# shincling/DL4SS

Measured on AMD Instinct MI355X. Metric: mixtures/sec (8 kHz, 4 s, 2-spk WSJ0-shape) at 1/2/4/8 MI355X, higher is better.
Workload: dtype bf16; 1 GPU; C2: 2-spk pit BiLSTM-4L magnitude mask (EvalVer model), B=32/GPU, N=32000 (T=251,F=129); global_batch=32, seq_len=251, parallelism=dp1, precision=bf16, loss=pit, launch=hip-graph, step=mix+STFT+fwd+loss+bwd+allreduce+Adam

## Files before the change

dl4ss_amd/_lib.py:

```python
import ctypes
import os

import torch

_HERE = os.path.dirname(os.path.abspath(__file__))
LIB_PATH = os.environ.get("DL4SS_LIB", os.path.join(_HERE, "libdl4ss_hip.so"))

P = ctypes.c_void_p
I = ctypes.c_int
LL = ctypes.c_longlong
F = ctypes.c_float
U = ctypes.c_uint

SIGNATURES = {
    "dl4ss_stft_fwd": [P, LL, I, I, I, I, P, P, P],
    "dl4ss_stft_fwd_ex": [P, LL, I, I, I, I, P, P, P, LL, LL, P],
    "dl4ss_istft": [P, LL, I, I, I, I, P, P],
    "dl4ss_mix_sources": [P, P, I, I, I, P, P, P, P],
    "dl4ss_gemm": [I, I, I, I, I, P, LL, P, LL, P, LL, P, I, F, I, I, P],
    "dl4ss_f32_to_bf16": [P, P, LL, P],
    "dl4ss_f32_to_bf16_2d": [P, LL, I, I, P, LL, P],
    "dl4ss_f32_to_bf16_hilo": [P, LL, I, I, P, LL, I, I, U, P],
    "dl4ss_birnn_bias_reduce": [I, I, I, I, P, P, P, P],
    "dl4ss_birnn_bias_reduce_ex": [I, I, I, I, P, P, P, F, P],
# ... 31 lines not shown
    "dl4ss_attn_dot_nblk": [I],
    "dl4ss_attn_dot_fwd": [P, P, I, I, I, I, I, P, P],
    "dl4ss_attn_dot_bwd": [P, P, I, P, P, I, I, I, I, P, P, P, P],
    "dl4ss_top_k_mask": [P, I, I, F, I, P, P, P, P],
    "dl4ss_attn_dot_fwd_ex": [P, P, I, I, I, I, I, P, LL, P],
    "dl4ss_classifier_select": [P, I, I, F, I, P, I, P, P, P, P],
    "dl4ss_mask_split": [P, P, LL, P, P, P],
    "dl4ss_time_mean": [P, I, I, I, P, P],
    "dl4ss_bss_corr": [P, I, I, I, I, P, P],
    "dl4ss_mix_sources_ex": [P, P, P, I, I, I, P, P, P, P],
    "dl4ss_mix_sources_rot": [P, P, P, P, I, I, I, P, P, P, P],
    "dl4ss_f32_to_bf16_2d_multi": [I, P, P, P, P, P, P, P],
    "dl4ss_mask_attn_loss_bf16v": [I, I, I, I, I, I, I, P, P, P, LL, P, LL, LL, P, F, F, P, P, LL, P, P, P, P, P],
    "dl4ss_bss_gram": [P, I, I, I, I, P, P, P, P],
    "dl4ss_adam_guarded": [P, P, P, P, LL, F, F, F, F, I, P, P, P],
    "dl4ss_adam_guarded_dp": [P, P, P, P, LL, F, F, F, F, I, P, P, P, P],
    "dl4ss_adam_guarded_dp_scaled": [P, P, P, P, LL, F, F, F, F, I, P, P, F, P, P],
    "dl4ss_adam_guarded_dp_scaled_bf16": [P, P, P, P, LL, F, F, F, F, I, P, P, F, P, I, P, P, P, P, P, P],
    "dl4ss_status_flag": [P, P, P],
    "dl4ss_birnn_plan_info": [I, I, I, I, I, P],
    "dl4ss_debug_set_spin_limit": [ctypes.c_uint],
    "dl4ss_debug_set_place_force": [ctypes.c_int],
    "dl4ss_debug_set_rnn_max_wg": [ctypes.c_int],
    "dl4ss_attn_align_nblk": [I],
    "dl4ss_attn_align_part_floats": [I, I, I],
    "dl4ss_attn_align_fwd": [P, P, I, P, P, P, I, I, I, P, LL, P],
    "dl4ss_attn_align_bwd": [P, P, I, P, P, P, P, I, I, I, P, P, LL, P, P, P, P, P],
    "dl4ss_mask_attn_align_loss": [I, I, I, I, I, I, P, P, P, P, P, P, LL, P, LL, LL, P, F, F, P, P, P, LL, P, P, P],
    "dl4ss_attn_align_finalize": [P, LL, I, I, I, I, P, P, P, P, P, P, P],
    "dl4ss_cls_head_fwd": [P, P, P, I, I, I, P, P, P],
    "dl4ss_cls_head_loss_bwd": [P, P, P, P, I, I, I, I, P, P, P, P, P, P],
    "dl4ss_disc_dims": [I, I, P],
    "dl4ss_disc_ws_bytes": [I, I, I],
    "dl4ss_disc_conv1_fwd": [I, P, P, P, I, I, I, P, P],
    "dl4ss_disc_conv64_fwd": [I, P, P, P, I, I, I, P, P],
    "dl4ss_disc_head_fwd": [I, P, P, P, I, I, I, P, P, P],
    "dl4ss_disc_head_bwd": [I, P, P, P, P, F, I, I, I, P, P, P, P, P, P],
    "dl4ss_disc_conv64_bwd": [I, P, P, P, P, I, I, I, P, P, P, P, LL, P],
    "dl4ss_disc_conv1_bwd": [I, P, P, P, P, I, I, I, P, P, P, P, LL, P],
}
RESTYPES = {"dl4ss_birnn_workspace_bytes": ctypes.c_longlong, "dl4ss_colsum_bf16_part_bytes": ctypes.c_longlong,
            "dl4ss_gemm_bf16_gl_ws_bytes": ctypes.c_longlong,
            "dl4ss_gemm_bf16_gl_grouped_ws_bytes": ctypes.c_longlong, "dl4ss_attn_nblk": ctypes.c_int,
            "dl4ss_attn_dot_nblk": ctypes.c_int, "dl4ss_attn_align_nblk": ctypes.c_int,
            "dl4ss_attn_align_part_floats": ctypes.c_longlong, "dl4ss_disc_ws_bytes": ctypes.c_longlong,
            "dl4ss_debug_set_spin_limit": None,
            "dl4ss_debug_set_place_force": None, "dl4ss_debug_set_rnn_max_wg": None}

_lib = None


def _load():
    global _lib
    if _lib is not None:
        return _lib
    if not os.path.exists(LIB_PATH):
        raise RuntimeError(
            f"dl4ss HIP library not found at {LIB_PATH}; run `python -m dl4ss_amd.build` "
            "(there is no CPU fallback)")
    lib = ctypes.CDLL(LIB_PATH)
    for name, argtypes in SIGNATURES.items():
        fn = getattr(lib, name)
        fn.argtypes = argtypes
        fn.restype = RESTYPES.get(name, ctypes.c_int)
    hip = ctypes.CDLL("libamdhip64.so")
    hip.hipGetErrorString.restype = ctypes.c_char_p
    hip.hipGetErrorString.argtypes = [ctypes.c_int]
    lib._hip = hip
    _lib = lib
    return lib
# ... 37 lines not shown
```

dl4ss_amd/csrc/birnn.hip:

```cpp
#include <cstdlib>
#include "birnn_common.h"

using namespace dl4ss_rnn;

namespace {

constexpr int DL4SS_RNN_WS_ZEROED = 0x100;
constexpr int DL4SS_RNN_DEFER_BIAS = 0x400;
constexpr int DL4SS_RNN_DGH_PAD8 = 0x200;
constexpr int DL4SS_RNN_DOUT_SLABS_MASK = 0x3000;
constexpr unsigned SPIN_LIMIT = 1u << 20;

struct Plan {
  int cell, H;
  int BC, NG, J, nchunk;
  int KP, KPL, HP, RP, RPL, KG, KGL;
  bool fwd_pk;
  bool bwd_pk;
  bool big;
  int R() const { return (cell == CELL_LSTM ? 4 : 3) * J; }
  int hm() const { return big ? HMAX_L : HMAX; }
  long long groups() const { return 2LL * nchunk; }
  size_t smem_fwd(bool mf) const { return fwd_lds_bytes(mf, hm(), BC, J, R(), HP, KP); }
  size_t smem_bwd(bool mf) const {
    int rpln, kgln;
    bwd_dims(RPL, KGL, rpln, kgln, big);
    return bwd_lds_bytes(mf, hm(), BC, J, NG, RP, RP * rpln, KG * kgln);
  }
  size_t smem_fwd_pk(bool xw) const { return fwd_pk_lds_bytes(BC, R(), xw); }
  size_t smem_bwd_pk() const { return bwd_pk_lds_bytes(BC, J); }
  long long zero_fwd(bool pk) const {
    return pk ? granule_bytes(groups(), PK_NCOPY, fwd_pk_copy_g(BC, NG)) : granule_bytes(groups(), GEN_NCOPY, fwd_copies_g(1, BC, H));
  }
  long long zero_bwd(bool pk) const {
    return pk ? granule_bytes(groups(), PK_NCOPY, bwd_pk_copy_g(BC, NG, H)) : granule_bytes(groups(), GEN_NCOPY, bwd_copies_g(1, BC, NG, H));
  }
};

int g_max_wg = 0;
int wg_limit() {
  if (g_max_wg > 0) return g_max_wg;
  static const int env = std::getenv("DL4SS_RNN_MAX_WG") ? std::atoi(std::getenv("DL4SS_RNN_MAX_WG")) : 0;
  if (env > 0) return env;
  const int cu = device_cu_count();
  return cu > 0 ? cu - cu / 16 : 240;
}

bool make_plan(int cell, int B, int H, Plan& p, bool mf = true, int max_wg = 0) {
  if (H > HMAX_L) return false;
  if (max_wg <= 0) max_wg = wg_limit();
  p.cell = cell;
  p.H = H;
  p.big = H > HMAX;
// ... 36 lines not shown
  return false;
}

bool act_cell_major(const Plan& p) { return p.fwd_pk && p.bwd_pk && p.BC >= 4; }

#if defined(RNN_STAMPS) || defined(RNN_TRACE)
u64* g_stamps = nullptr;
#endif

unsigned g_spin_limit = SPIN_LIMIT;
int g_place_force = 0;

void fill_args(RnnArgs& a, const Plan& p, int B, int T, int H) {
  a.spin_limit = g_spin_limit;
  a.place_force = g_place_force;
#if defined(RNN_STAMPS) || defined(RNN_TRACE)
  a.stamps = g_stamps;
#endif
  a.B = B; a.T = T; a.H = H; a.J = p.J; a.NG = p.NG; a.nchunk = p.nchunk;
  a.KP = p.KP; a.KPL = p.KPL; a.HP = p.HP;
  a.RP = p.RP; a.RPL = p.RPL; a.KG = p.KG; a.KGL = p.KGL;
}

int launch(bool fwd, bool mf, bool pk, const Plan& p, const RnnArgs& a, size_t smem, hipStream_t st) {
  const int grid = (int)(p.groups() * p.NG);
  const int e = fwd ? (pk ? launch_fwd_pk(a, p.cell, p.BC, grid, smem, st) : launch_fwd(a, p.cell, p.BC, mf, grid, smem, st))
                    : (pk ? launch_bwd_pk(a, p.cell, p.BC, grid, smem, st) : launch_bwd(a, p.cell, p.BC, mf, grid, smem, st));
  if (e) return e;
  DL4SS_CHECK_LAUNCH();
  return 0;
}

}

#if defined(RNN_STAMPS) || defined(RNN_TRACE)
DL4SS_API void dl4ss_debug_set_stamps(void* p) { g_stamps = reinterpret_cast<unsigned long long*>(p); }
#endif

constexpr int BIAS_JOBS_MAX = 8;
struct BiasJobs {
  int n, B, GH;
  float beta;
  const float* part[BIAS_JOBS_MAX];
  float* dbi[BIAS_JOBS_MAX];
  float* dbh[BIAS_JOBS_MAX];
};
__global__ __launch_bounds__(256) void bias_reduce_kernel(BiasJobs j) {
  const int i = blockIdx.x * 256 + threadIdx.x;
  const int B = j.B, GH = j.GH;
  if (i >= 2 * GH) return;
// ... 22 lines not shown
  }
  if (dbi) dbi[i] = j.beta != 0.f ? si + j.beta * dbi[i] : si;
  if (dbh) dbh[i] = j.beta != 0.f ? sh + j.beta * dbh[i] : sh;
}

static long long handoff_bytes(const Plan& p, int H);

static long long bias_part_bytes(const Plan& p, int H) {
  return p.big ? 0 : (long long)p.nchunk * p.BC * 2 * 2 * 4 * H * 4;
}

static long long workspace_bytes(const Plan& p, int H) { return handoff_bytes(p, H) + bias_part_bytes(p, H); }

static long long handoff_bytes(const Plan& p, int H) { return handoff_area_bytes(p.groups(), p.BC, p.NG, H, p.big); }

static long long ctl_offset(const Plan& p, int H) { return ctl_offset_bytes(p.groups(), p.BC, p.NG, H); }

DL4SS_API void dl4ss_debug_set_spin_limit(unsigned limit) { g_spin_limit = limit ? limit : SPIN_LIMIT; }

DL4SS_API void dl4ss_debug_set_place_force(int force) { g_place_force = force == 1 ? 1 : 0; }

DL4SS_API void dl4ss_debug_set_rnn_max_wg(int max_wg) { g_max_wg = max_wg > 0 ? max_wg : 0; }

DL4SS_API int dl4ss_birnn_plan_info(int cell, int B, int H, int precision, int max_wg, int* info) {
  DL4SS_REQUIRE(info && (cell == CELL_LSTM || cell == CELL_GRU) && B > 0 && H > 0);
  Plan p;
  if (!make_plan(cell, B, H, p, precision == 1, max_wg)) return (int)hipErrorInvalidValue;
  info[0] = p.BC; info[1] = p.NG; info[2] = p.J; info[3] = p.nchunk; info[4] = 2 * p.nchunk * p.NG;
  return 0;
}

static int split_batch(int cell, int B, int H, bool mf, Plan& ps) {
  int fit = 0;
  for (int b = B - 1; b >= 1 && !fit; --b)
    if (make_plan(cell, b, H, ps, mf)) fit = b;
  if (!fit) return 0;
  const int n = (B + fit - 1) / fit;
  const int bs = (B + n - 1) / n;
  return make_plan(cell, bs, H, ps, mf) ? bs : 0;
}

DL4SS_API long long dl4ss_birnn_workspace_bytes(int cell, int B, int H) {
  long long best = -1;
  for (bool mf : {false, true}) {
    Plan p;
    if (!make_plan(cell, B, H, p, mf) && (mf || split_batch(cell, B, H, mf, p) == 0)) continue;
// ... 198 lines not shown
  DL4SS_REQUIRE(dOut || !pk);
  DL4SS_REQUIRE(pk || (!dG_bf16 && !dGh_bf16 && !db_ih && !db_hh && dG && (cell == CELL_LSTM || dGh)));
  DL4SS_REQUIRE(dout_ns == 1 || (pk && p.BC == 4));
  if (!prezeroed) {
    hipError_t e = hipMemsetAsync(workspace, 0, p.zero_bwd(pk), st);
    if (e == hipSuccess && pk) e = hipMemsetAsync(static_cast<char*>(workspace) + ctl_offset(p, H), 0, CTL_BYTES, st);
    if (e != hipSuccess) return (int)e;
  }
  RnnArgs a{};
  fill_args(a, p, B, T, H);
  a.Whh = W_hh; a.act = const_cast<float*>(act); a.cs = const_cast<float*>(cs);
  a.hprev = const_cast<float*>(hprev); a.dOut = dOut; a.dOutB = dOut_bcast; a.dG = dG; a.dGh = dGh;
  a.dout_ns = dout_ns;
  a.dout_zs = (long long)B * T * 2 * H;
  a.dGb = reinterpret_cast<unsigned short*>(dG_bf16); a.dGhb = reinterpret_cast<unsigned short*>(dGh_bf16);
  const int GHc = (cell == CELL_LSTM ? 4 : 3) * H;
  a.ghb = dgh_pad8 ? (GHc + 7) / 8 * 8 : GHc;
  a.dbi = db_ih; a.dbh = db_hh;
  a.xbuf = reinterpret_cast<unsigned long long*>(workspace);
  a.gctl = pk ? reinterpret_cast<unsigned*>(static_cast<char*>(workspace) + ctl_offset(p, H)) : nullptr;
  const bool bias = pk && (db_ih || db_hh);
  a.dbpart = bias ? reinterpret_cast<float*>(static_cast<char*>(workspace) + handoff_bytes(p, H)) : nullptr;
  a.status = status;
  const int e = launch(false, mf, pk, p, a, pk ? p.smem_bwd_pk() : p.smem_bwd(mf), st);
  if (e || !bias || defer_bias) return e;
  const int GH = (cell == CELL_LSTM ? 4 : 3) * H;
  BiasJobs j{};
  j.n = 1; j.B = B; j.GH = GH; j.beta = 1.f; j.part[0] = a.dbpart; j.dbi[0] = db_ih; j.dbh[0] = db_hh;
  hipLaunchKernelGGL(bias_reduce_kernel, dim3((2 * GH + 255) / 256, 1), dim3(256), 0, st, j);
  return (int)hipGetLastError();
}

DL4SS_API int dl4ss_birnn_bias_reduce_ex(int cell, int B, int H, int n, void* const* workspaces,
                                         float* const* db_ih, float* const* db_hh, float beta, void* stream) {
  DL4SS_REQUIRE((cell == CELL_LSTM || cell == CELL_GRU) && B > 0 && H > 0 && n >= 1 && n <= BIAS_JOBS_MAX);
  DL4SS_REQUIRE(workspaces && db_ih && db_hh);
  Plan p;
  if (!make_plan(cell, B, H, p, true)) return (int)hipErrorInvalidValue;
  const int GH = (cell == CELL_LSTM ? 4 : 3) * H;
  BiasJobs j{};
  j.n = n; j.B = B; j.GH = GH; j.beta = beta;
  for (int i = 0; i < n; ++i) {
    DL4SS_REQUIRE(workspaces[i] && db_ih[i] && db_hh[i]);
    j.part[i] = reinterpret_cast<const float*>(static_cast<const char*>(workspaces[i]) + handoff_bytes(p, H));
    j.dbi[i] = db_ih[i];
    j.dbh[i] = db_hh[i];
  }
// ... 11 lines not shown
```

dl4ss_amd/csrc/birnn_bwd_pk.hip:

```cpp
#include "birnn_common.h"

namespace dl4ss_rnn {

__device__ __forceinline__ unsigned pack24(float v) {
  const unsigned u = __float_as_uint(v);
  return (u + 0x80u) >> 8;
}
__device__ __forceinline__ float unpack24(unsigned r) { return __uint_as_float(r << 8); }

template <int CELL, int BC, int NZ = 1>
__global__ __launch_bounds__(NT, 1) void rnn_bwd_pk_kernel(RnnArgs a) {
  constexpr int NGATE = CELL == CELL_LSTM ? 4 : 3;
  constexpr int BSL_Q = BC * 5;
  constexpr int BSL_G = 64 / BSL_Q > 0 ? 64 / BSL_Q : 1;
  constexpr int BSL_N = BWD_NPW * BSL_G < 16 ? BWD_NPW * BSL_G : 16;
  constexpr int GLK = (16 + BSL_N - 1) / BSL_N;
  static_assert(BSL_Q <= 64, "one (b, quad) item per lane");
  constexpr int WSPAN = bwd_wspan(HMAX);
  constexpr int MTWMAX = WSPAN / 16;
  constexpr int KSRMAX = (4 * JMAX + 31) / 32;
  constexpr int WSP = BWD_PK_WSP;
  const int H = a.H, T = a.T, J = a.J, NG = a.NG;
  const int R = NGATE * J;
  const int ngroups = 2 * a.nchunk;
  extern __shared__ __attribute__((aligned(16))) float smem[];
  int group, w;
  group_pk(a.gctl, NG, ngroups, a.spin_limit, a.status, smem, group, w);
  const int d = group / a.nchunk, chunk = group % a.nchunk;
  const int b0 = chunk * BC;
  const int j0 = w * J;
  const int tid = threadIdx.x;
  const int lane = tid & 63, wv = tid >> 6;
  const int GH = NGATE * H;
  const int AH = 4 * H;
  const int HG = ((H + 1) / 2 + 1) & ~1;

  unsigned short* sdgb = reinterpret_cast<unsigned short*>(smem);
  float* sdh = smem + 8 * SDG;
  float* wsc = sdh + ((16 * BC * J + 3) & ~3);
  constexpr int SOPP = bwd_pk_sopp(BC);
  constexpr int WSCN = bwd_pk_wsc_n(BC), SOPN = bwd_pk_sop_n(BC);
  float* sop = wsc + WSCN;
  for (int i = tid; i < 8 * SDG + 16 * BC * J; i += NT) smem[i] = 0.0f;

  const bool mv = wv < 4;
  bf16x8 afr[MTWMAX][KSRMAX];
#pragma unroll
  for (int t = 0; t < MTWMAX; ++t) {
    const int k = (wv * MTWMAX + t) * 16 + (lane & 15);
#pragma unroll
    for (int ks = 0; ks < KSRMAX; ++ks)
#pragma unroll
      for (int j = 0; j < 8; ++j) {
        const int rr = ks * 32 + 8 * (lane >> 4) + j;
        const int q = rr / J, u = rr % J;
        const bool ok = mv && k < H && rr < R && j0 + u < H;
        afr[t][ks][j] = (short)bf16_rne(ok ? a.Whh[((long long)d * GH + q * H + j0 + u) * H + k] : 0.0f);
      }
  }

  const int cb = tid >> 5, cu = tid & 31;
  const bool ct = tid < BC * 32 && cu < J;
  const int cj = j0 + cu;
  const int bg = b0 + cb;
  const bool cval = ct && cj < H && bg < a.B;
  float dc_next = 0.0f, dh_dir = 0.0f;
  const float doutb = (cval && a.dOutB) ? a.dOutB[(long long)bg * 2 * H + d * H + cj] : 0.0f;

  const int copy_g = NG * BC * HG;
  u64* xg = a.xbuf + (long long)group * PK_NCOPY * copy_g;
  const __amdgpu_buffer_rsrc_t xr = granule_rsrc(xg, (unsigned)(PK_NCOPY * copy_g * 8));
  __shared__ int s_wt;
  if (tid == 0) __hip_atomic_store(xg + PK_PLACE_COPY * copy_g + w, (1ull << 32) | xcc_id(), __ATOMIC_RELAXED, __HIP_MEMORY_SCOPE_AGENT);
  if (wv == WPOLL) {
    const bool wt = group_needs_write_through(xg + PK_PLACE_COPY * copy_g, NG, lane, a.spin_limit, a.status, a.place_force);
    if (lane == 0) s_wt = wt;
  }

  constexpr int WPF = WPOLL + BWD_NPW;
  constexpr int NPF = NT - WPF * 64;
  constexpr int NSL = CELL == CELL_LSTM ? 7 : 6;
// ... 115 lines not shown
      const int p = sl + BSL_N * g;
      on[g] = lane_on && p < NG;
      loff[g] = on[g] ? (p * BC + pb_b) * HG + (j0 >> 1) + 2 * qd : 0;
    }
    const int doff = lane_on ? (sl * BC + pb_b) * J + 4 * qd : 0;
    for (int s = 0; s < T; ++s) {
      if (s > 0) {
        const unsigned tag = (unsigned)s & 0xFFFFu;
        if (wv == WPOLL) TRACE(2, s);
        const int sb = ((s - 1) & 1) * 2 * copy_g * 8;
        u32x4 q[GLK], qa[GLK], qb[GLK];
        unsigned done = 0;
        asm volatile("" ::: "memory");
#pragma unroll
        for (int g = 0; g < GLK; ++g) qa[g] = __builtin_amdgcn_raw_buffer_load_b128(xr, sb + loff[g] * 8, 0, 16);
        unsigned spins = 0;
        while (true) {
          asm volatile("" ::: "memory");
#pragma unroll
          for (int g = 0; g < GLK; ++g) qb[g] = __builtin_amdgcn_raw_buffer_load_b128(xr, sb + loff[g] * 8, 0, 16);
#pragma unroll
          for (int g = 0; g < GLK; ++g) {
            const bool m = ((qa[g].y >> 16) == tag) & ((qa[g].w >> 16) == tag) & !((done >> g) & 1);
            q[g] = m ? qa[g] : q[g];
            done |= (unsigned)m << g;
          }
          if (done == (1u << GLK) - 1) break;
          asm volatile("" ::: "memory");
#pragma unroll
          for (int g = 0; g < GLK; ++g) qa[g] = __builtin_amdgcn_raw_buffer_load_b128(xr, sb + loff[g] * 8, 0, 16);
#pragma unroll
          for (int g = 0; g < GLK; ++g) {
            const bool m = ((qb[g].y >> 16) == tag) & ((qb[g].w >> 16) == tag) & !((done >> g) & 1);
            q[g] = m ? qb[g] : q[g];
            done |= (unsigned)m << g;
          }
          if (done == (1u << GLK) - 1) break;
          if (++spins > a.spin_limit) {
            atomicOr(a.status, 2);
            return;
          }
        }
        float4 acc4 = make_float4(0.f, 0.f, 0.f, 0.f);
#pragma unroll
        for (int g = 0; g < GLK; ++g) {
          if (on[g]) {
            const unsigned l0 = q[g].x, l1 = q[g].y, h0 = q[g].z, h1 = q[g].w;
            acc4.x += unpack24(l0 & 0xFFFFFFu);
            acc4.y += unpack24((l0 >> 24) | ((l1 & 0xFFFFu) << 8));
            acc4.z += unpack24(h0 & 0xFFFFFFu);
            acc4.w += unpack24((h0 >> 24) | ((h1 & 0xFFFFu) << 8));
          }
        }
        if (lane_on) *reinterpret_cast<float4*>(sdh + doff) = acc4;
        if (wv == WPOLL) TRACE(1, s);
      }
      STAMP(0)
// ... 43 lines not shown
        const int tn = tstep(min(s + 2, T - 1));
        L.issue(tn, T);
        act_issue(A, tn);
        __syncthreads();
      };
      int s = 0;
      for (; s + 1 < T; s += 2) {
        pf_step(s, ld, av);
        pf_step(s + 1, ld2, av2);
      }
      if (s < T) pf_step(s, ld, av);
    } else {
      for (int s = 0; s < T; ++s) {
        ld.commit(sop + (s & 1) * 2 * SOPP);
        __syncthreads();
        if (s + 1 < T) ld.issue(tstep(s + 1), T);
        __syncthreads();
        if (s + 1 == T) break;
      }
    }
    return;
  }

  float sbi[NGATE], sbh[NGATE];
  float pgi[NGATE], pgh[NGATE];
  int pt = 0;
#pragma unroll
  for (int q = 0; q < NGATE; ++q) sbi[q] = sbh[q] = pgi[q] = pgh[q] = 0.0f;
  auto store_dg = [&]() {
    if (!cval) return;
    const long long go = (long long)((bg * T + pt) * 2 + d) * GH + cj;
    if (a.dG) {
#pragma unroll
      for (int q = 0; q < NGATE; ++q) a.dG[go + q * H] = pgi[q];
    }
    if (a.dGb) {
#pragma unroll
      for (int q = 0; q < NGATE; ++q) a.dGb[go + q * H] = bf16_rne(pgi[q]);
    }
    if (CELL == CELL_GRU) {
      if (a.dGh) {
#pragma unroll
        for (int q = 0; q < NGATE; ++q) a.dGh[go + q * H] = pgh[q];
      }
      if (a.dGhb) {
        const long long goh = (long long)((bg * T + pt) * 2 + d) * a.ghb + cj;
// ... 199 lines not shown
    store_dg();
#endif
    STAMP(6)
  }
  if (cval && a.dbpart) {
    float* pp = a.dbpart + (long long)(bg * 2 + d) * 2 * GH;
#pragma unroll
    for (int q = 0; q < NGATE; ++q) {
      pp[q * H + cj] = sbi[q];
      pp[GH + q * H + cj] = sbh[q];
    }
  } else if (cval) {
#pragma unroll
    for (int q = 0; q < NGATE; ++q) {
      if (a.dbi) atomicAdd(a.dbi + d * GH + q * H + cj, sbi[q]);
      if (a.dbh) atomicAdd(a.dbh + d * GH + q * H + cj, sbh[q]);
    }
  }
  STAMP_FLUSH
}

namespace {
template <int CELL, int BC>
int launch_bwd_pk_t(const RnnArgs& a, int grid, size_t smem, hipStream_t st) {
  if constexpr (BC == 4) {
    if (a.dout_ns == 2) return launch_resident(rnn_bwd_pk_kernel<CELL, 4, 2>, grid, smem, st, a);
    if (a.dout_ns == 3) return launch_resident(rnn_bwd_pk_kernel<CELL, 4, 3>, grid, smem, st, a);
    if (a.dout_ns == 4) return launch_resident(rnn_bwd_pk_kernel<CELL, 4, 4>, grid, smem, st, a);
  }
  return launch_resident(rnn_bwd_pk_kernel<CELL, BC>, grid, smem, st, a);
}
template <int CELL>
int launch_bwd_pk_c(const RnnArgs& a, int BC, int grid, size_t smem, hipStream_t st) {
  switch (BC) {
#ifndef RNN_EXP_MINIMAL
    case 1: return launch_bwd_pk_t<CELL, 1>(a, grid, smem, st);
    case 2: return launch_bwd_pk_t<CELL, 2>(a, grid, smem, st);
    case 8: return launch_bwd_pk_t<CELL, 8>(a, grid, smem, st);
#endif
    case 4: return launch_bwd_pk_t<CELL, 4>(a, grid, smem, st);
    default: return (int)hipErrorInvalidValue;
  }
}
}

int launch_bwd_pk(const RnnArgs& a, int cell, int BC, int grid, size_t smem, hipStream_t st) {
  if (a.H > HMAX) return (int)hipErrorInvalidValue;
  return cell == CELL_LSTM ? launch_bwd_pk_c<CELL_LSTM>(a, BC, grid, smem, st)
                           : launch_bwd_pk_c<CELL_GRU>(a, BC, grid, smem, st);
}

}
```

dl4ss_amd/csrc/birnn_common.h:

```cpp
#pragma once
#include <mutex>
#include <type_traits>
#include "birnn_layout.h"
#include "common.h"

namespace dl4ss_rnn __attribute__((visibility("hidden"))) {

enum { CELL_LSTM = 0, CELL_GRU = 1 };

typedef unsigned long long u64;

#ifdef RNN_STAMPS
__device__ __forceinline__ u64 stamp_now() {
  u64 t;
  __builtin_amdgcn_sched_barrier(0);
  asm volatile("s_memtime %0\n\ts_waitcnt lgkmcnt(0)" : "=s"(t)::"memory");
  __builtin_amdgcn_sched_barrier(0);
  return t;
}
#define STAMP_DECL u64 st_prev = stamp_now(), st_acc[8] = {0, 0, 0, 0, 0, 0, 0, 0};
#define STAMP(i) { const u64 n_ = stamp_now(); st_acc[i] += n_ - st_prev; st_prev = n_; }
#ifndef STAMP_T2
#define STAMP_T2 NROLE
#endif
// ... 182 lines not shown
    for (int g = 0; g < GM; ++g) ok &= (unsigned)(v[g] >> 32) == tag;
    if (ok) return true;
    if (++spins > limit) return false;
    __builtin_amdgcn_s_sleep(1);
#pragma unroll
    for (int g = 0; g < GM; ++g)
      if ((unsigned)(v[g] >> 32) != tag) v[g] = get_granule(src + off[g]);
  }
}

typedef unsigned u32x4 __attribute__((ext_vector_type(4)));
constexpr int WPOLL = 4;
constexpr int BWD_NPW = 2;
constexpr int FWD_MV_CHAINS = 2;
constexpr int FWD_NPW = 2;
static_assert(FWD_MV_CHAINS >= 1 && FWD_MV_CHAINS <= 8, "FWD_MV_CHAINS: 1..KSMAX accumulator chains");
static_assert(FWD_NPW >= 1 && FWD_NPW <= 3, "FWD_NPW: 1..3 polling waves");
static_assert(BWD_NPW >= 1 && BWD_NPW <= 3, "BWD_NPW: 1..3 polling waves");

__device__ __forceinline__ __amdgpu_buffer_rsrc_t granule_rsrc(const void* p, unsigned bytes) {
  return __builtin_amdgcn_make_buffer_rsrc(const_cast<void*>(p), 0, bytes, 0x00020000);
}

__device__ __forceinline__ unsigned xcc_id() {
  unsigned x;
  asm volatile("s_getreg_b32 %0, hwreg(HW_REG_XCC_ID)" : "=s"(x));
  return x & 0xFu;
}

__device__ __forceinline__ void group_pk(unsigned* ctl, int NG, int ngroups, unsigned limit, int* status, float* smem,
                                         int& group, int& w) {
  if (ctl == nullptr || (ngroups & 7) != 0) {
    group_of(blockIdx.x, NG, ngroups, group, w);
    return;
  }
  int* sg = reinterpret_cast<int*>(smem);
  if (threadIdx.x == 0) {
    const int per = ngroups >> 3, cap = per * NG, nwg = ngroups * NG;
    const unsigned x = xcc_id() & 7u;
    const int slot = (int)__hip_atomic_fetch_add(ctl + x, 1u, __ATOMIC_RELAXED, __HIP_MEMORY_SCOPE_AGENT);
    int g = -1, m = 0;
    if (slot < cap) {
      g = (int)x * per + slot / NG;
      m = slot % NG;
    } else {
      const int ov = (int)__hip_atomic_fetch_add(ctl + 8, 1u, __ATOMIC_RELAXED, __HIP_MEMORY_SCOPE_AGENT);
// ... 73 lines not shown
    kgln = 4;
  } else if (!big && ((rpl == 20 && kgl == 3) || (rpl == 20 && kgl == 2))) {
    rpln = rpl;
    kgln = kgl;
  } else {
    rpln = RPLMAX;
    kgln = KGLMAX;
  }
}

inline int device_cu_count() {
  static int cache[64] = {0};
  int dev = 0;
  if (hipGetDevice(&dev) != hipSuccess || dev < 0 || dev >= 64) return 0;
  if (cache[dev] == 0) {
    int cu = 0;
    if (hipDeviceGetAttribute(&cu, hipDeviceAttributeMultiprocessorCount, dev) != hipSuccess) return 0;
    cache[dev] = cu;
  }
  return cache[dev];
}

template <typename K>
bool fits_resident(K kernel, int grid, size_t smem) {
  struct Entry { const void* k; size_t smem; int dev; int occ; };
  static std::mutex mu;
  static Entry cache[64];
  static int n = 0;
  int dev = 0;
  if (hipGetDevice(&dev) != hipSuccess) return false;
  const void* kp = reinterpret_cast<const void*>(kernel);
  std::lock_guard<std::mutex> lk(mu);
  int occ = -1;
  for (int i = 0; i < n; ++i)
    if (cache[i].k == kp && cache[i].smem == smem && cache[i].dev == dev) occ = cache[i].occ;
  if (occ < 0) {
    occ = 0;
    if (hipOccupancyMaxActiveBlocksPerMultiprocessor(&occ, kernel, NT, smem) != hipSuccess) occ = 0;
    if (n < 64) cache[n++] = Entry{kp, smem, dev, occ};
  }
  return grid <= occ * device_cu_count();
}

template <typename K>
int launch_resident(K kernel, int grid, size_t smem, hipStream_t st, const RnnArgs& a) {
  if (!fits_resident(kernel, grid, smem)) return (int)hipErrorCooperativeLaunchTooLarge;
  RnnArgs arg = a;
  void* args[] = {&arg};
  return (int)hipLaunchKernel(reinterpret_cast<const void*>(kernel), dim3(grid), dim3(NT), args, smem, st);
}

int launch_fwd(const RnnArgs& a, int cell, int BC, bool mf, int grid, size_t smem, hipStream_t st);
int launch_fwd_pk(const RnnArgs& a, int cell, int BC, int grid, size_t smem, hipStream_t st);
int launch_bwd(const RnnArgs& a, int cell, int BC, bool mf, int grid, size_t smem, hipStream_t st);
int launch_bwd_pk(const RnnArgs& a, int cell, int BC, int grid, size_t smem, hipStream_t st);

}
```

dl4ss_amd/csrc/birnn_layout.h:

```cpp
#pragma once
#include <hip/hip_runtime.h>

namespace dl4ss_rnn {

#define RNN_HD __host__ __device__ constexpr

constexpr int NT = 512;
constexpr int NROLE = 256;
constexpr int JMAX = 20;
constexpr int WMAX = 64;
constexpr int RPLMAX = 20;
constexpr int KGLMAX = 6;
constexpr int HMAX = 320;
constexpr int HMAX_L = 640;
constexpr int LDS_BYTES = 160 * 1024;

RNN_HD int shb_stride(int hm) { return hm / 32 * 32 + 8; }
constexpr int SDG = (4 * JMAX + 31) / 32 * 32 + 8;
RNN_HD int mfma_tiles(int R) { return (R + 15) / 16; }
RNN_HD int bwd_wspan(int hm) { return (hm / 16 + 3) / 4 * 16; }
RNN_HD int round4(int n) { return (n + 3) & ~3; }

RNN_HD int fwd_sh_n(int BC, int HP) { return BC * HP; }
RNN_HD int fwd_spart_n(int KP, int BC, int R) { return KP * BC * R; }
// ... 24 lines not shown
RNN_HD int xw_ring_bf16(int bc) { return 3 * xw_spb(bc) * xw_slot(bc); }
RNN_HD int fwd_pk_nsin(int bc, bool xw) { return xw ? 2 * xw_spb(bc) : 2; }
RNN_HD int fwd_pk_sgs(int R) { return mfma_tiles(R) * 16 + 4; }
RNN_HD int fwd_pk_sgate_n(int BC, int R) { return BC * fwd_pk_sgs(R); }
RNN_HD int fwd_pk_sgx_n(int BC) { return BC * 16; }
RNN_HD int fwd_pk_sin_n(int BC, bool xw) { return fwd_pk_nsin(BC, xw) * sin_slab(BC); }
RNN_HD int fwd_pk_spub_bf16(int BC) { return BC * PKU; }
RNN_HD size_t fwd_pk_lds_bytes(int BC, int R, bool xw) {
  return sizeof(float) * (size_t)(fwd_shb_n(HMAX) + fwd_pk_sgate_n(BC, R) + fwd_pk_sgx_n(BC) + fwd_pk_sin_n(BC, xw)) +
         sizeof(unsigned short) * (size_t)fwd_pk_spub_bf16(BC) +
         (xw ? 256 + sizeof(unsigned short) * (size_t)xw_ring_bf16(BC) : 0);
}

constexpr int BWD_PK_WSP = bwd_wspan(HMAX) + 4;
RNN_HD int bwd_pk_sopp(int bc) { return bc * 32 * 4 + 16; }
RNN_HD int bwd_pk_cpwp(int bc) { return (bc * JMAX + 1) / 2; }
RNN_HD int bwd_pk_sdh_n(int BC, int J) { return round4(16 * BC * J); }
RNN_HD int bwd_pk_wsc_n(int BC) { return 4 * BC * BWD_PK_WSP; }
RNN_HD int bwd_pk_sop_n(int BC) { return 2 * 2 * bwd_pk_sopp(BC); }
RNN_HD int bwd_pk_sraw_n(int BC) { return 2 * 7 * bwd_pk_cpwp(BC); }
RNN_HD size_t bwd_pk_lds_bytes(int BC, int J) {
  return sizeof(float) * (size_t)(8 * SDG + bwd_pk_sdh_n(BC, J) + bwd_pk_wsc_n(BC) + bwd_pk_sop_n(BC) + bwd_pk_sraw_n(BC));
}

constexpr int GEN_NCOPY = 2, PK_NCOPY = 4, PK_PLACE_COPY = 3;
constexpr int CTL_BYTES = 256;
RNN_HD int pk_hg(int H) { return ((H + 1) / 2 + 1) & ~1; }
RNN_HD long long fwd_copies_g(long long n, int BC, int H) { return n * BC * H; }
RNN_HD int fwd_pk_copy_g(int BC, int NG) { return BC * NG * 8; }
RNN_HD long long bwd_copies_g(long long n, int BC, int NG, int H) { return n * NG * BC * H; }
RNN_HD int bwd_pk_copy_g(int BC, int NG, int H) { return NG * BC * pk_hg(H); }
RNN_HD long long granule_bytes(long long groups, int ncopy, long long copy_g) { return groups * ncopy * copy_g * 8; }
RNN_HD long long max2(long long a, long long b) { return a > b ? a : b; }
RNN_HD long long handoff_area_bytes(long long groups, int BC, int NG, int H, bool big) {
  long long n = max2(granule_bytes(groups, GEN_NCOPY, fwd_copies_g(1, BC, H)), granule_bytes(groups, GEN_NCOPY, bwd_copies_g(1, BC, NG, H)));
  if (!big)
    n = max2(n, max2(granule_bytes(groups, PK_NCOPY, fwd_pk_copy_g(BC, NG)), granule_bytes(groups, PK_NCOPY, bwd_pk_copy_g(BC, NG, H))));
  return (n + 255) / 256 * 256 + (big ? 0 : CTL_BYTES);
}
RNN_HD long long ctl_offset_bytes(long long groups, int BC, int NG, int H) {
  return handoff_area_bytes(groups, BC, NG, H, false) - CTL_BYTES;
}

RNN_HD bool lds_fits_all_bc(int which) {
  constexpr int R = 4 * JMAX, NG = HMAX_L / JMAX;
  for (int bc = 1; bc <= 8; bc *= 2) {
// ... 19 lines not shown
```

include/dl4ss_hip.h:

```cpp
#ifndef DL4SS_HIP_H
#define DL4SS_HIP_H

#ifdef __cplusplus
extern "C" {
#endif

enum {
  DL4SS_STFT_COMPLEX = 1,
  DL4SS_STFT_MAG = 2,
  DL4SS_STFT_LOGMAG = 4,
  DL4SS_STFT_CONJ = 8
};

int dl4ss_stft_fwd(const float* x, long long n_sig, int n_samples, int n_fft, int hop, int flags,
                   float* X_c64, float* mag, void* stream);
int dl4ss_stft_fwd_ex(const float* x, long long n_sig, int n_samples, int n_fft, int hop, int flags, float* X_c64,
                      float* mag, void* mag_bf16, long long ld_bf16, long long n_sig_bf16, void* stream);

int dl4ss_istft(const float* S_c64, long long n_sig, int T, int n_fft, int hop, int flags, float* y,
                void* stream);
int dl4ss_istft_apply(const float* X_mix_c64, const float* aux, long long n_sig, int k_per_mix, int T, int mode,
                      int conj, float* y, void* stream);

int dl4ss_mix_sources(const float* raw, const float* gains, int B, int K, int N, float* stats_ws, float* out_src,
// ... 33 lines not shown
int dl4ss_colsum_bf16(const void* A, long long lda, int M, int N, float* out, void* stream);
long long dl4ss_colsum_bf16_part_bytes(int M, int N);
int dl4ss_colsum_bf16_det(const void* A, long long lda, int M, int N, float* out, float* part, long long part_bytes,
                          void* stream);
int dl4ss_colsum_bf16_det_ex(const void* A, long long lda, int M, int N, float* out, float* part,
                             long long part_bytes, float beta, void* stream);
int dl4ss_f32_to_bf16_2d_multi(int n, const float* const* x, const long long* ldx, const int* rows, const int* cols,
                               void* const* y, const long long* ldy, void* stream);

enum { DL4SS_CELL_LSTM = 0, DL4SS_CELL_GRU = 1 };
#define DL4SS_RNN_WS_ZEROED 0x100
#define DL4SS_RNN_DGH_PAD8 0x200
#define DL4SS_RNN_DEFER_BIAS 0x400
#define DL4SS_RNN_DOUT_SLABS(S) ((((S) - 1) & 3) << 12)
int dl4ss_birnn_bias_reduce(int cell, int B, int H, int n, void* const* workspaces, float* const* db_ih,
                            float* const* db_hh, void* stream);
int dl4ss_birnn_bias_reduce_ex(int cell, int B, int H, int n, void* const* workspaces, float* const* db_ih,
                               float* const* db_hh, float beta, void* stream);
long long dl4ss_birnn_workspace_bytes(int cell, int B, int H);
int dl4ss_birnn_plan_info(int cell, int B, int H, int precision, int max_wg, int* info);
void dl4ss_debug_set_spin_limit(unsigned limit);
void dl4ss_debug_set_place_force(int force);
void dl4ss_debug_set_rnn_max_wg(int max_wg);
int dl4ss_birnn_fwd(int cell, int precision, int B, int T, int H, const float* G, const float* W_hh,
                    const float* b_hh, float* out, float* hprev, float* act, float* cs, void* workspace,
                    long long ws_bytes, int* status, void* stream);
int dl4ss_birnn_fwd_ex(int cell, int precision, int B, int T, int H, const float* G, const float* W_hh,
                       const float* b_hh, float* out, float* hprev, float* act, float* cs, void* out_bf16,
                       void* hprev_bf16, void* workspace, long long ws_bytes, int* status, void* stream);
int dl4ss_birnn_fwd_mean(int cell, int precision, int B, int T, int H, const float* G, const float* W_hh,
                         const float* b_hh, float* out, float* hprev, float* act, float* cs, void* out_bf16,
                         void* hprev_bf16, float* h_mean, void* workspace, long long ws_bytes, int* status, void* stream);
int dl4ss_birnn_fwd_xw(int cell, int B, int T, int H, const void* x_bf16, int Kin, long long ldx,
                       const void* W_ih_bf16, long long ldw, const float* b_ih, const float* W_hh,
                       const float* b_hh, float* out, float* hprev, float* act, float* cs, void* out_bf16,
                       void* hprev_bf16, void* workspace, long long ws_bytes, int* status, void* stream,
                       int ws_zeroed);
int dl4ss_birnn_fwd_xw_ex(int cell, int B, int T, int H, const void* x_bf16, int Kin, long long ldx,
                          const void* W_ih_bf16, long long ldw, const float* b_ih, const float* W_hh, const float* b_hh,
                          float* out, float* hprev, float* act, float* cs, void* out_bf16, void* hprev_bf16,
                          float* h_mean, void* workspace, long long ws_bytes, int* status, void* stream, int ws_zeroed);
int dl4ss_birnn_fwd_xw_supported(int cell, int B, int T, int H, int Kin);
int dl4ss_birnn_bwd(int cell, int precision, int B, int T, int H, const float* dOut, const float* dOut_bcast,
                    const float* W_hh, const float* act, const float* cs, const float* hprev, float* dG, float* dGh, void* workspace,
                    long long ws_bytes, int* status, void* stream);

// ... 108 lines not shown
```

Measured before the change: 9617 mixtures/s.

## Add two-workgroups-per-CU variant of packed BiRNN backward kernel for LSTM

Adds a W2 variant of the persistent packed RNN backward kernel that targets two resident workgroups per CU. It raises waves_per_eu, caps LDS at half the CU, and requires a minimum occupancy of 2 at launch. To cut register pressure, the bf16 recurrent weight fragments are loaded after the setup phase instead of up front. LSTM defaults to two per CU, and an env var and debug setter can override this. The intent is more latency hiding in the recurrent backward pass, at the cost of register spills or LDS contention and the risk that the cooperative launch fails if occupancy cannot be met.

```diff
diff --git a/dl4ss_amd/_lib.py b/dl4ss_amd/_lib.py
--- a/dl4ss_amd/_lib.py
+++ b/dl4ss_amd/_lib.py
@@ -77,6 +77,9 @@
     "dl4ss_debug_set_spin_limit": [ctypes.c_uint],
     "dl4ss_debug_set_place_force": [ctypes.c_int],
     "dl4ss_debug_set_rnn_max_wg": [ctypes.c_int],
+    "dl4ss_debug_set_rnn_bwd_per_cu": [ctypes.c_int],
+    "dl4ss_debug_set_rnn_place_out": [P],
+    "dl4ss_birnn_bwd_plan_info": [I, I, I, I, I, P],
     "dl4ss_attn_align_nblk": [I],
     "dl4ss_attn_align_part_floats": [I, I, I],
     "dl4ss_attn_align_fwd": [P, P, I, P, P, P, I, I, I, P, LL, P],
@@ -100,7 +103,8 @@
             "dl4ss_attn_dot_nblk": ctypes.c_int, "dl4ss_attn_align_nblk": ctypes.c_int,
             "dl4ss_attn_align_part_floats": ctypes.c_longlong, "dl4ss_disc_ws_bytes": ctypes.c_longlong,
             "dl4ss_debug_set_spin_limit": None,
-            "dl4ss_debug_set_place_force": None, "dl4ss_debug_set_rnn_max_wg": None}
+            "dl4ss_debug_set_place_force": None, "dl4ss_debug_set_rnn_max_wg": None,
+            "dl4ss_debug_set_rnn_bwd_per_cu": None, "dl4ss_debug_set_rnn_place_out": None}
 
 _lib = None
 
diff --git a/dl4ss_amd/csrc/birnn.hip b/dl4ss_amd/csrc/birnn.hip
--- a/dl4ss_amd/csrc/birnn.hip
+++ b/dl4ss_amd/csrc/birnn.hip
@@ -29,6 +29,8 @@
   }
   size_t smem_fwd_pk(bool xw) const { return fwd_pk_lds_bytes(BC, R(), xw); }
   size_t smem_bwd_pk() const { return bwd_pk_lds_bytes(BC, J); }
+  bool bwd_w2() const { return bwd_pk && bwd_pk2_fits(BC, J); }
+  size_t smem_bwd_pk2() const { return bwd_pk2_lds_bytes(BC, J); }
   long long zero_fwd(bool pk) const {
     return pk ? granule_bytes(groups(), PK_NCOPY, fwd_pk_copy_g(BC, NG)) : granule_bytes(groups(), GEN_NCOPY, fwd_copies_g(1, BC, H));
   }
@@ -111,10 +113,18 @@
   a.RP = p.RP; a.RPL = p.RPL; a.KG = p.KG; a.KGL = p.KGL;
 }
 
-int launch(bool fwd, bool mf, bool pk, const Plan& p, const RnnArgs& a, size_t smem, hipStream_t st) {
+int g_bwd_per_cu = 0;
+int bwd_per_cu(int cell) {
+  if (g_bwd_per_cu > 0) return g_bwd_per_cu;
+  static const int env = std::getenv("DL4SS_RNN_BWD_PER_CU") ? std::atoi(std::getenv("DL4SS_RNN_BWD_PER_CU")) : 0;
+  if (env == 1 || env == 2) return env;
+  return cell == CELL_LSTM ? 2 : 1;
+}
+
+int launch(bool fwd, bool mf, bool pk, const Plan& p, const RnnArgs& a, size_t smem, hipStream_t st, bool w2 = false) {
   const int grid = (int)(p.groups() * p.NG);
   const int e = fwd ? (pk ? launch_fwd_pk(a, p.cell, p.BC, grid, smem, st) : launch_fwd(a, p.cell, p.BC, mf, grid, smem, st))
-                    : (pk ? launch_bwd_pk(a, p.cell, p.BC, grid, smem, st) : launch_bwd(a, p.cell, p.BC, mf, grid, smem, st));
+                    : (pk ? launch_bwd_pk(a, p.cell, p.BC, w2, grid, smem, st) : launch_bwd(a, p.cell, p.BC, mf, grid, smem, st));
   if (e) return e;
   DL4SS_CHECK_LAUNCH();
   return 0;
@@ -183,6 +193,22 @@
 
 DL4SS_API void dl4ss_debug_set_rnn_max_wg(int max_wg) { g_max_wg = max_wg > 0 ? max_wg : 0; }
 
+DL4SS_API void dl4ss_debug_set_rnn_bwd_per_cu(int n) { g_bwd_per_cu = n == 1 || n == 2 ? n : 0; }
+
+unsigned long long* g_place_out = nullptr;
+DL4SS_API void dl4ss_debug_set_rnn_place_out(void* p) { g_place_out = reinterpret_cast<unsigned long long*>(p); }
+
+DL4SS_API int dl4ss_birnn_bwd_plan_info(int cell, int B, int H, int max_wg, int per_cu, int* info) {
+  DL4SS_REQUIRE(info && (cell == CELL_LSTM || cell == CELL_GRU) && B > 0 && H > 0 && (per_cu == 1 || per_cu == 2));
+  Plan p;
+  if (!make_plan(cell, B, H, p, true, max_wg) || !p.bwd_pk) return (int)hipErrorInvalidValue;
+  if (per_cu == 2 && !p.bwd_w2()) return (int)hipErrorCooperativeLaunchTooLarge;
+  const int grid = 2 * p.nchunk * p.NG;
+  info[0] = per_cu; info[1] = grid; info[2] = (grid + per_cu - 1) / per_cu;
+  info[3] = (int)(per_cu == 2 ? p.smem_bwd_pk2() : p.smem_bwd_pk());
+  return 0;
+}
+
 DL4SS_API int dl4ss_birnn_plan_info(int cell, int B, int H, int precision, int max_wg, int* info) {
   DL4SS_REQUIRE(info && (cell == CELL_LSTM || cell == CELL_GRU) && B > 0 && H > 0);
   Plan p;
@@ -427,7 +453,11 @@
   const bool bias = pk && (db_ih || db_hh);
   a.dbpart = bias ? reinterpret_cast<float*>(static_cast<char*>(workspace) + handoff_bytes(p, H)) : nullptr;
   a.status = status;
-  const int e = launch(false, mf, pk, p, a, pk ? p.smem_bwd_pk() : p.smem_bwd(mf), st);
+  const bool w2 = pk && bwd_per_cu(cell) == 2 && p.bwd_w2();
+#if !defined(RNN_STAMPS) && !defined(RNN_TRACE)
+  if (w2) a.stamps = g_place_out;
+#endif
+  const int e = launch(false, mf, pk, p, a, pk ? (w2 ? p.smem_bwd_pk2() : p.smem_bwd_pk()) : p.smem_bwd(mf), st, w2);
   if (e || !bias || defer_bias) return e;
   const int GH = (cell == CELL_LSTM ? 4 : 3) * H;
   BiasJobs j{};
diff --git a/dl4ss_amd/csrc/birnn_bwd_pk.hip b/dl4ss_amd/csrc/birnn_bwd_pk.hip
--- a/dl4ss_amd/csrc/birnn_bwd_pk.hip
+++ b/dl4ss_amd/csrc/birnn_bwd_pk.hip
@@ -8,8 +8,13 @@
 }
 __device__ __forceinline__ float unpack24(unsigned r) { return __uint_as_float(r << 8); }
 
-template <int CELL, int BC, int NZ = 1>
-__global__ __launch_bounds__(NT, 1) void rnn_bwd_pk_kernel(RnnArgs a) {
+constexpr int BWD_PK_W2 = 0x100;
+template <int CELL, int BCX, int NZ = 1>
+__global__ __launch_bounds__(NT) __attribute__((amdgpu_waves_per_eu(BCX >= BWD_PK_W2 ? 4 : 2)))
+void rnn_bwd_pk_kernel(RnnArgs a) {
+  constexpr int BC = BCX & (BWD_PK_W2 - 1);
+  constexpr bool W2 = BCX >= BWD_PK_W2;
+  static_assert(!W2 || BC == 4, "the two-per-CU family exists at BC = 4");
   constexpr int NGATE = CELL == CELL_LSTM ? 4 : 3;
   constexpr int BSL_Q = BC * 5;
   constexpr int BSL_G = 64 / BSL_Q > 0 ? 64 / BSL_Q : 1;
@@ -26,11 +31,21 @@
   extern __shared__ __attribute__((aligned(16))) float smem[];
   int group, w;
   group_pk(a.gctl, NG, ngroups, a.spin_limit, a.status, smem, group, w);
+  if constexpr (W2) {
+    group = __builtin_amdgcn_readfirstlane(group);
+    w = __builtin_amdgcn_readfirstlane(w);
+  }
   const int d = group / a.nchunk, chunk = group % a.nchunk;
   const int b0 = chunk * BC;
   const int j0 = w * J;
   const int tid = threadIdx.x;
   const int lane = tid & 63, wv = tid >> 6;
+#if !defined(RNN_STAMPS) && !defined(RNN_TRACE)
+  if constexpr (W2) {
+    if (a.stamps && tid == 0)
+      a.stamps[blockIdx.x] = ((u64)(group * 16 + w + 1) << 40) | ((u64)xcc_id() << 32) | hw_id();
+  }
+#endif
   const int GH = NGATE * H;
   const int AH = 4 * H;
   const int HG = ((H + 1) / 2 + 1) & ~1;
@@ -45,6 +60,7 @@
 
   const bool mv = wv < 4;
   bf16x8 afr[MTWMAX][KSRMAX];
+  if constexpr (!W2) {
 #pragma unroll
   for (int t = 0; t < MTWMAX; ++t) {
     const int k = (wv * MTWMAX + t) * 16 + (lane & 15);
@@ -57,6 +73,7 @@
         const bool ok = mv && k < H && rr < R && j0 + u < H;
         afr[t][ks][j] = (short)bf16_rne(ok ? a.Whh[((long long)d * GH + q * H + j0 + u) * H + k] : 0.0f);
       }
+  }
   }
 
   const int cb = tid >> 5, cu = tid & 31;
@@ -218,7 +235,12 @@
 #pragma unroll
           for (int g = 0; g < GLK; ++g) {
             const bool m = ((qa[g].y >> 16) == tag) & ((qa[g].w >> 16) == tag) & !((done >> g) & 1);
-            q[g] = m ? qa[g] : q[g];
+            if constexpr (W2 && CELL == CELL_GRU) {
+              const unsigned mm = 0u - (unsigned)m;
+              q[g] = (qa[g] & mm) | (q[g] & ~mm);
+            } else {
+              q[g] = m ? qa[g] : q[g];
+            }
             done |= (unsigned)m << g;
           }
           if (done == (1u << GLK) - 1) break;
@@ -228,7 +250,12 @@
 #pragma unroll
           for (int g = 0; g < GLK; ++g) {
             const bool m = ((qb[g].y >> 16) == tag) & ((qb[g].w >> 16) == tag) & !((done >> g) & 1);
-            q[g] = m ? qb[g] : q[g];
+            if constexpr (W2 && CELL == CELL_GRU) {
+              const unsigned mm = 0u - (unsigned)m;
+              q[g] = (qb[g] & mm) | (q[g] & ~mm);
+            } else {
+              q[g] = m ? qb[g] : q[g];
+            }
             done |= (unsigned)m << g;
           }
           if (done == (1u << GLK) - 1) break;
@@ -318,6 +345,48 @@
     return;
   }
 
+  if constexpr (W2) {
+    const float* wb = a.Whh + (long long)d * GH * H;
+    const int kb = wv * WSPAN + (lane & 15);
+#pragma unroll
+    for (int ks = 0; ks < KSRMAX; ++ks) {
+      const int rr0 = ks * 32 + 8 * (lane >> 4);
+      int q = rr0 / J, u = rr0 - q * J;
+      unsigned ro[8], pm[4];
+#pragma unroll
+      for (int j = 0; j < 8; ++j) {
+        const bool rok = rr0 + j < R && j0 + u < H;
+        ro[j] = rok ? (unsigned)((q * H + j0 + u) * H) : 0u;
+        const unsigned m = rok ? (j & 1 ? 0xFFFF0000u : 0xFFFFu) : 0u;
+        pm[j >> 1] = j & 1 ? pm[j >> 1] | m : m;
+        if (++u == J) {
+          u = 0;
+          ++q;
+        }
+      }
+#pragma unroll
+      for (int ta = 0; ta < MTWMAX; ta += 3) {
+        float wf[3][8];
+#pragma unroll
+        for (int t = ta; t < ta + 3 && t < MTWMAX; ++t) {
+          unsigned kk = (unsigned)min(kb + 16 * t, H - 1);
+          asm volatile("" : "+v"(kk));
+#pragma unroll
+          for (int j = 0; j < 8; ++j) wf[t - ta][j] = wb[ro[j] + kk];
+        }
+#pragma unroll
+        for (int t = ta; t < ta + 3 && t < MTWMAX; ++t) {
+          const unsigned km = kb + 16 * t < H ? 0xFFFFFFFFu : 0u;
+          u32x4 pw;
+#pragma unroll
+          for (int j = 0; j < 8; j += 2)
+            pw[j >> 1] = ((unsigned)bf16_rne(wf[t - ta][j]) | ((unsigned)bf16_rne(wf[t - ta][j + 1]) << 16)) & pm[j >> 1] & km;
+          asm volatile("" : "+v"(pw));
+          afr[t][ks] = __builtin_bit_cast(bf16x8, pw);
+        }
+      }
+    }
+  }
   float sbi[NGATE], sbh[NGATE];
   float pgi[NGATE], pgh[NGATE];
   int pt = 0;
@@ -563,7 +632,16 @@
 
 namespace {
 template <int CELL, int BC>
-int launch_bwd_pk_t(const RnnArgs& a, int grid, size_t smem, hipStream_t st) {
+int launch_bwd_pk_t(const RnnArgs& a, bool wg2, int grid, size_t smem, hipStream_t st) {
+  if constexpr (BC == 4) {
+    if (wg2) {
+      if (a.dout_ns == 2) return launch_resident(rnn_bwd_pk_kernel<CELL, 4 + BWD_PK_W2, 2>, grid, smem, st, a, 2);
+      if (a.dout_ns == 3) return launch_resident(rnn_bwd_pk_kernel<CELL, 4 + BWD_PK_W2, 3>, grid, smem, st, a, 2);
+      if (a.dout_ns == 4) return launch_resident(rnn_bwd_pk_kernel<CELL, 4 + BWD_PK_W2, 4>, grid, smem, st, a, 2);
+      return launch_resident(rnn_bwd_pk_kernel<CELL, 4 + BWD_PK_W2, 1>, grid, smem, st, a, 2);
+    }
+  }
+  if (wg2) return (int)hipErrorInvalidValue;
   if constexpr (BC == 4) {
     if (a.dout_ns == 2) return launch_resident(rnn_bwd_pk_kernel<CELL, 4, 2>, grid, smem, st, a);
     if (a.dout_ns == 3) return launch_resident(rnn_bwd_pk_kernel<CELL, 4, 3>, grid, smem, st, a);
@@ -572,23 +650,23 @@
   return launch_resident(rnn_bwd_pk_kernel<CELL, BC>, grid, smem, st, a);
 }
 template <int CELL>
-int launch_bwd_pk_c(const RnnArgs& a, int BC, int grid, size_t smem, hipStream_t st) {
+int launch_bwd_pk_c(const RnnArgs& a, int BC, bool wg2, int grid, size_t smem, hipStream_t st) {
   switch (BC) {
 #ifndef RNN_EXP_MINIMAL
-    case 1: return launch_bwd_pk_t<CELL, 1>(a, grid, smem, st);
-    case 2: return launch_bwd_pk_t<CELL, 2>(a, grid, smem, st);
-    case 8: return launch_bwd_pk_t<CELL, 8>(a, grid, smem, st);
+    case 1: return launch_bwd_pk_t<CELL, 1>(a, wg2, grid, smem, st);
+    case 2: return launch_bwd_pk_t<CELL, 2>(a, wg2, grid, smem, st);
+    case 8: return launch_bwd_pk_t<CELL, 8>(a, wg2, grid, smem, st);
 #endif
-    case 4: return launch_bwd_pk_t<CELL, 4>(a, grid, smem, st);
+    case 4: return launch_bwd_pk_t<CELL, 4>(a, wg2, grid, smem, st);
     default: return (int)hipErrorInvalidValue;
   }
 }
 }
 
-int launch_bwd_pk(const RnnArgs& a, int cell, int BC, int grid, size_t smem, hipStream_t st) {
+int launch_bwd_pk(const RnnArgs& a, int cell, int BC, bool wg2, int grid, size_t smem, hipStream_t st) {
   if (a.H > HMAX) return (int)hipErrorInvalidValue;
-  return cell == CELL_LSTM ? launch_bwd_pk_c<CELL_LSTM>(a, BC, grid, smem, st)
-                           : launch_bwd_pk_c<CELL_GRU>(a, BC, grid, smem, st);
+  return cell == CELL_LSTM ? launch_bwd_pk_c<CELL_LSTM>(a, BC, wg2, grid, smem, st)
+                           : launch_bwd_pk_c<CELL_GRU>(a, BC, wg2, grid, smem, st);
 }
 
 }
diff --git a/dl4ss_amd/csrc/birnn_common.h b/dl4ss_amd/csrc/birnn_common.h
--- a/dl4ss_amd/csrc/birnn_common.h
+++ b/dl4ss_amd/csrc/birnn_common.h
@@ -228,6 +228,12 @@
   return __builtin_amdgcn_make_buffer_rsrc(const_cast<void*>(p), 0, bytes, 0x00020000);
 }
 
+__device__ __forceinline__ unsigned hw_id() {
+  unsigned x;
+  asm volatile("s_getreg_b32 %0, hwreg(HW_REG_HW_ID)" : "=s"(x));
+  return x;
+}
+
 __device__ __forceinline__ unsigned xcc_id() {
   unsigned x;
   asm volatile("s_getreg_b32 %0, hwreg(HW_REG_XCC_ID)" : "=s"(x));
@@ -347,7 +353,7 @@
 }
 
 template <typename K>
-bool fits_resident(K kernel, int grid, size_t smem) {
+bool fits_resident(K kernel, int grid, size_t smem, int min_occ = 1) {
   struct Entry { const void* k; size_t smem; int dev; int occ; };
   static std::mutex mu;
   static Entry cache[64];
@@ -364,12 +370,12 @@
     if (hipOccupancyMaxActiveBlocksPerMultiprocessor(&occ, kernel, NT, smem) != hipSuccess) occ = 0;
     if (n < 64) cache[n++] = Entry{kp, smem, dev, occ};
   }
-  return grid <= occ * device_cu_count();
+  return occ >= min_occ && grid <= occ * device_cu_count();
 }
 
 template <typename K>
-int launch_resident(K kernel, int grid, size_t smem, hipStream_t st, const RnnArgs& a) {
-  if (!fits_resident(kernel, grid, smem)) return (int)hipErrorCooperativeLaunchTooLarge;
+int launch_resident(K kernel, int grid, size_t smem, hipStream_t st, const RnnArgs& a, int min_occ = 1) {
+  if (!fits_resident(kernel, grid, smem, min_occ)) return (int)hipErrorCooperativeLaunchTooLarge;
   RnnArgs arg = a;
   void* args[] = {&arg};
   return (int)hipLaunchKernel(reinterpret_cast<const void*>(kernel), dim3(grid), dim3(NT), args, smem, st);
@@ -378,6 +384,6 @@
 int launch_fwd(const RnnArgs& a, int cell, int BC, bool mf, int grid, size_t smem, hipStream_t st);
 int launch_fwd_pk(const RnnArgs& a, int cell, int BC, int grid, size_t smem, hipStream_t st);
 int launch_bwd(const RnnArgs& a, int cell, int BC, bool mf, int grid, size_t smem, hipStream_t st);
-int launch_bwd_pk(const RnnArgs& a, int cell, int BC, int grid, size_t smem, hipStream_t st);
-
-}
+int launch_bwd_pk(const RnnArgs& a, int cell, int BC, bool wg2, int grid, size_t smem, hipStream_t st);
+
+}
diff --git a/dl4ss_amd/csrc/birnn_layout.h b/dl4ss_amd/csrc/birnn_layout.h
--- a/dl4ss_amd/csrc/birnn_layout.h
+++ b/dl4ss_amd/csrc/birnn_layout.h
@@ -70,6 +70,10 @@
 RNN_HD size_t bwd_pk_lds_bytes(int BC, int J) {
   return sizeof(float) * (size_t)(8 * SDG + bwd_pk_sdh_n(BC, J) + bwd_pk_wsc_n(BC) + bwd_pk_sop_n(BC) + bwd_pk_sraw_n(BC));
 }
+RNN_HD size_t bwd_pk2_lds_bytes(int BC, int J) {
+  return bwd_pk_lds_bytes(BC, J) > (size_t)(LDS_BYTES / 2 - 1024) ? bwd_pk_lds_bytes(BC, J) : (size_t)(LDS_BYTES / 2 - 1024);
+}
+RNN_HD bool bwd_pk2_fits(int BC, int J) { return BC == 4 && 2 * (bwd_pk2_lds_bytes(BC, J) + 1024) <= (size_t)LDS_BYTES; }
 
 constexpr int GEN_NCOPY = 2, PK_NCOPY = 4, PK_PLACE_COPY = 3;
 constexpr int CTL_BYTES = 256;
diff --git a/include/dl4ss_hip.h b/include/dl4ss_hip.h
--- a/include/dl4ss_hip.h
+++ b/include/dl4ss_hip.h
@@ -79,6 +79,9 @@
 void dl4ss_debug_set_spin_limit(unsigned limit);
 void dl4ss_debug_set_place_force(int force);
 void dl4ss_debug_set_rnn_max_wg(int max_wg);
+void dl4ss_debug_set_rnn_bwd_per_cu(int n);
+void dl4ss_debug_set_rnn_place_out(void* p);
+int dl4ss_birnn_bwd_plan_info(int cell, int B, int H, int max_wg, int per_cu, int* info);
 int dl4ss_birnn_fwd(int cell, int precision, int B, int T, int H, const float* G, const float* W_hh,
                     const float* b_hh, float* out, float* hprev, float* act, float* cs, void* workspace,
                     long long ws_bytes, int* status, void* stream);
```

Result: no change. 9682 mixtures/s, median of 6 (+0.7%).
